# lhaippp/DMHomo

Hardware: AMD Instinct MI355X
Metric: sampled images/sec (128x128, s_step=32) (higher is better)
Workload: dtype f32; 1 GPU; DGM CFG-Unet dim=64 128x128 bs=25/GPU s_step=32 cond_scale=3 (BASELINE configs[1]); global_batch=25, cfg_mode=streams, hip_graph=True, weights=seeded random init

## Files before the change

### dmhomo_amd/_lib.py

```python
import contextlib
import ctypes as C
import gc
import os

import torch

_HERE = os.path.dirname(os.path.abspath(__file__))
LIB_PATH = os.environ.get('DMH_LIB_PATH') or os.path.join(_HERE, 'libdmhomo_hip.so')

c_f32p = C.c_void_p
c_i64 = C.c_int64
c_int = C.c_int
c_float = C.c_float


ABI_VERSION = 500


class DmhConv(C.Structure):
    _fields_ = [('struct_size', C.c_uint64)] + \
               [(n, C.c_void_p) for n in ('src0', 'src1', 'wpack', 'bias', 'in_coef', 'res', 'res_coef', 'out',
                                          'stats')] + \
               [(n, C.c_int32) for n in ('B', 'Hin', 'Win', 'C0', 'C1', 'Cout', 'KH', 'KW', 'stride', 'upsample2')] + \
               [('in_bound', C.c_void_p), ('in_bound_n', C.c_int32), ('fin_n', C.c_int32), ('fin_w', C.c_void_p),
                ('fin_b', C.c_void_p), ('fin_out', C.c_void_p), ('pix_stats', C.c_void_p), ('pix_eps', C.c_float),
                ('rows', C.c_void_p)]


class DmhPackJob(C.Structure):
    _fields_ = [('src', C.c_void_p), ('ws', C.c_void_p), ('wpack', C.c_void_p), ('Cout', C.c_int32), ('C0', C.c_int32),
                ('C1', C.c_int32), ('KH', C.c_int32), ('transposed', C.c_int32)]


class DmhStep(C.Structure):
    _fields_ = [('objective', C.c_int32), ('clip', C.c_int32), ('mode', C.c_int32), ('cond_scale', C.c_float),
                ('sqrt_recip_ac', C.c_float), ('sqrt_recipm1_ac', C.c_float), ('sqrt_ac', C.c_float),
                ('sqrt_1m_ac', C.c_float), ('c0', C.c_float), ('c1', C.c_float), ('c2', C.c_float)]


SIGNATURES = {
    'dmh_last_error': (C.c_char_p, []),
    'dmh_version': (c_int, []),
    'dmh_ws_standardize': (c_int, [c_f32p, c_f32p, c_int, c_int, c_float, C.c_void_p]),
    'dmh_conv_pack_floats': (c_i64, [c_int, c_int, c_int, c_int, c_int]),
    'dmh_pack_conv_weight': (c_int, [c_f32p, c_f32p, c_int, c_int, c_int, c_int, c_int, C.c_void_p]),
    'dmh_pack_conv_weights_multi': (c_int, [C.c_void_p, c_int, c_float, C.c_void_p]),
# ... 158 lines not shown
    'dmh_preview_sheet': (c_int, [c_f32p, c_f32p, c_f32p, C.c_void_p, C.c_void_p, c_int, c_int, c_int, c_int, c_int, c_int,
                                  C.c_void_p]),
    'dmh_homography_warp': (c_int, [c_f32p, C.c_void_p, c_f32p, c_int, c_int, c_int, c_int, c_int, C.c_void_p]),
    'dmh_hem_batch': (c_int, [C.c_void_p, C.c_void_p, C.c_void_p, C.c_void_p, C.c_void_p, C.c_void_p, c_int, c_int, c_int, c_int,
                              c_int, c_int, c_int, c_f32p, c_f32p, c_f32p, c_f32p, c_f32p, C.c_void_p]),
    'dmh_hem_flow': (c_int, [C.c_void_p, c_int, c_int, c_int, c_f32p, C.c_void_p]),
}

EXTENSIONS = {
    'dmh_known_blend': (c_int, [c_f32p, c_f32p, C.c_void_p, c_float, c_f32p, C.c_void_p, c_f32p, c_int, c_i64, C.c_void_p]),
    'dmh_known_error_splits': (c_int, [c_int, c_i64]),
    'dmh_known_error': (c_int, [c_f32p, c_f32p, C.c_void_p, c_float, c_f32p, C.c_void_p, C.c_void_p, C.c_void_p, c_int, c_i64,
                                C.c_void_p]),
}

DLT_BLOCKS = 64

_lib = None


class DmhError(RuntimeError):
    pass


def lib():
    global _lib
    if _lib is None:
        if not os.path.exists(LIB_PATH):
            raise DmhError(f'{LIB_PATH} not found: build it with `python -c "import __graft_entry__ as g; g.build()"` '
                           f'or `make -C dmhomo_amd/csrc` — dmhomo_amd has no CPU / eager fallback')
        h = C.CDLL(LIB_PATH)
        for name, (res, args) in list(SIGNATURES.items()) + list(EXTENSIONS.items()):
            fn = getattr(h, name)
            fn.restype = res
            fn.argtypes = args
        got = int(h.dmh_version())
        if got != ABI_VERSION:
            raise DmhError(f'{LIB_PATH} reports ABI version {got}, this binding was written against {ABI_VERSION} '
                           f'(include/dmhomo_hip.h): rebuild the library with `make -C dmhomo_amd/csrc`')
        _lib = h
    return _lib


def stream():
    return C.c_void_p(torch.cuda.current_stream().cuda_stream)


# ... 31 lines not shown
```

### dmhomo_amd/cfg.py

```python
import torch
from torch import nn

from . import _params as P
from . import ops
from .engine import UnetEngine
from .sampling import DeviceRng, ModelPrediction, ScheduleHost, default, exists, extract
from .schedule import make_buffers, ddim_pairs, linear_beta_schedule, cosine_beta_schedule


class Unet(nn.Module):

    def __init__(self, dim, num_classes, cond_drop_prob=0.5, init_dim=None, out_dim=None, dim_mults=(1, 2, 4, 8),
                 channels=3, resnet_block_groups=8, learned_variance=False, learned_sinusoidal_cond=False,
                 random_fourier_features=False, learned_sinusoidal_dim=16):
        super().__init__()
        self.cond_drop_prob = cond_drop_prob
        self.channels = channels
        input_channels = channels + 3
        init_dim = default(init_dim, dim)
        self.init_conv = nn.Conv2d(input_channels, init_dim, 7, padding=3)
        time_dim = dim * 4
        self.random_or_learned_sinusoidal_cond = learned_sinusoidal_cond or random_fourier_features
        pos_emb, fourier_dim = P.time_embedding(dim, learned_sinusoidal_cond, random_fourier_features, learned_sinusoidal_dim)
        self.time_mlp = nn.Sequential(pos_emb, nn.Linear(fourier_dim, time_dim), nn.GELU(), nn.Linear(time_dim, time_dim))
# ... 25 lines not shown
        z = cache.get(key)
        if z is None:
            z = cache[key] = torch.zeros((batch,), device=device, dtype=torch.uint8)
        return z

    def _stem(self, x, rgb_flow, mask):
        if not x.is_cuda:
            raise RuntimeError('dmhomo_amd.Unet runs on the GPU only (HIP kernels); move the inputs with .cuda()')
        eng = self._engine
        eng.ensure_prepared()
        xin = ops.assemble_input(x.to(torch.float32).contiguous(), rgb_flow.to(torch.float32).contiguous(),
                                 mask.to(torch.float32).contiguous(), reps=1, cpad=eng.cin_pad)
        return eng.stem(xin)

    def _run(self, x, time, classes, rgb_flow, mask, keeps, taps=None, x0=None, first=None, out=None, rows=None,
             x0_per_pass=False, pert_lo=None):
        eng = self._engine
        if x0 is None:
            x0 = self._stem(x, rgb_flow, mask)
        if len(keeps) > 1 and not x0_per_pass:
            x0 = x0.repeat(len(keeps), 1, 1, 1)
        time = time.to(torch.int64).contiguous()
        classes = classes.to(torch.int64).contiguous()
        tab = self.__dict__.get('_ss_tab')
        if tab is not None:
            T, Ct, cursor = tab
            B = classes.shape[0]
            ss_all = torch.empty((len(keeps) * B, T.shape[1]), device=T.device, dtype=torch.float32)
            for r, k in enumerate(keeps):
                ops.ss_gather(T, Ct, eng.mlp_b, cursor, classes, k, out=ss_all[r * B:(r + 1) * B])
            return eng.trunk(x0, None, taps, first=first, out=out, ss_all=ss_all, rows=rows, pert_lo=pert_lo)
        cond = eng.embed(time, [(classes, k) for k in keeps], len(keeps))
        return eng.trunk(x0, cond, taps, first=first, out=out, rows=rows, pert_lo=pert_lo)

    def forward(self, x, time, classes, rgb_flow, mask, cond_drop_prob=None):
        cond_drop_prob = default(cond_drop_prob, self.cond_drop_prob)
        keep = self._keep_mask(x.shape[0], cond_drop_prob, x.device)
        return self._run(x, time, classes, rgb_flow, mask, [keep])

    cfg_mode = 'batched'
    stream_splits = 1

    def _cond_null(self, x, time, classes, rgb_flow, mask, gate=None):
        B = x.shape[0]
        keep = self._keep_mask(B, self.cond_drop_prob, x.device)
        null = self._null_mask(B, x.device)
        dedup = bool(self.dedup_dropped_rows) and keep is not None
        if self.cfg_mode == 'streams':
            nsub = max(1, min(int(self.stream_splits), B))
            nstreams = 2 * nsub
            if len(getattr(self, '_side', ())) != nstreams:
                self._side = tuple(torch.cuda.Stream(device=x.device) for _ in range(nstreams))
            cur = torch.cuda.current_stream()
            x0 = self._stem(x, rgb_flow, mask)
            first = self._engine.first_conv(x0)
            cond_out = torch.empty((B, self.out_dim) + tuple(x.shape[2:]), device=x.device, dtype=torch.float32)
            null_out = torch.empty_like(cond_out)
            bounds = [(i * B) // nsub for i in range(nsub + 1)]
            si = 0
            for k, dst, sub, null_side in ((keep, cond_out, dedup, False), (null, null_out, False, True)):
                for lo, hi in zip(bounds[:-1], bounds[1:]):
                    st = self._side[si]
                    si += 1
                    st.wait_stream(cur)
                    with torch.cuda.stream(st):
                        kk = None if k is None else k[lo:hi].contiguous()
                        fs = None if first is None else (first[0][lo:hi], first[1][lo:hi])
                        if gate is not None:
                            rows = ops.rows_gated(kk if sub else None, hi - lo, 0, *gate, null_side=null_side)
                        else:
                            rows = ops.rows_from_keep(kk) if sub else None
                        self._run(None, time[lo:hi], classes[lo:hi], None, None, [kk], x0=x0[lo:hi], first=fs, out=dst[lo:hi],
                                  rows=rows)
            for st in self._side:
                cur.wait_stream(st)
            return cond_out, null_out, (keep if dedup else None)
        if gate is not None:
            rows = ops.rows_gated(keep if dedup else None, B, B, *gate)
        else:
            rows = ops.rows_from_keep(keep, extra=B) if dedup else None
        both = self._run(x, time, classes, rgb_flow, mask, [keep, null], rows=rows)
        return both[:B], both[B:], (keep if dedup else None)

    def _cond_null_noflow(self, x, time, classes, rgb_flow, mask, cond_scale):
        if self.cfg_mode == 'streams':
            raise ValueError("flow_guidance with cfg_mode = 'streams': the third pass is defined for cfg_mode = 'batched' only")
        B, eng = x.shape[0], self._engine
        keep = self._keep_mask(B, self.cond_drop_prob, x.device)
# ... 635 lines not shown
```

### dmhomo_amd/csrc/common.h

```cpp
#pragma once
#include <initializer_list>
#include <hip/hip_runtime.h>
#include <stdint.h>
#include <stdio.h>

#include "../../include/dmhomo_hip.h"

void dmh_set_error(const char* fmt, ...);

#define DMH_REQUIRE(cond, ...)   \
  do {                           \
    if (!(cond)) {               \
      dmh_set_error(__VA_ARGS__); \
      return DMH_EINVAL;         \
    }                            \
  } while (0)

#define DMH_CHECK_LAUNCH(name)                                        \
  do {                                                                \
    hipError_t e_ = hipGetLastError();                                \
    if (e_ != hipSuccess) {                                           \
      dmh_set_error("%s: launch failed: %s", name, hipGetErrorString(e_)); \
      return DMH_ELAUNCH;                                             \
    }                                                                 \
// ... 125 lines not shown
```

### dmhomo_amd/csrc/conv.hip

```cpp
#include <stdlib.h>

#include "common.h"

#include "conv_args.h"
#include "weight_image.h"

template <int KH, int KW, int S, int UPS, int KC, int TH, int TW>
struct ConvCfg {
  static constexpr int BM = TH * TW;
  static constexpr int MB = BM / 128;
  static constexpr int IN_H = (TH - 1) * S + KH;
  static constexpr int IN_W = (TW - 1) * S + KW;
  static constexpr int IN_PIX = IN_H * IN_W;
  static constexpr int KCP = KC + 4;
  static constexpr int C4 = KC / 4;
  static constexpr int NLOAD = (IN_PIX * C4 + 255) / 256;
  static constexpr int WL = 64 * C4 / 256;
  static constexpr int PAD = (S == 1) ? (KH / 2) : (KH == 4 ? 1 : 0);
  static constexpr int IN_FLOATS = IN_PIX * KCP;
  static constexpr int W_FLOATS = 64 * KCP;
  static constexpr int EPI_BYTES = 4 * 32 * 68 * 4;
  static constexpr int MAIN_BYTES = (IN_FLOATS + 2 * W_FLOATS) * 4;
  static constexpr int LDS_BYTES = MAIN_BYTES > EPI_BYTES ? MAIN_BYTES : EPI_BYTES;
};
// ... 296 lines not shown
  DMH_REQUIRE(w && wpack && dmh_conv_up2_pack_floats(Cout, C0) > 0, "dmh_pack_conv_weight_up2: bad arguments");
  return dmh_f16x3_up2_pack(w, wpack, Cout, C0, (hipStream_t)stream);
}

extern "C" int dmh_pack_conv_weights_multi(const DmhPackJob* jobs, int njobs, float ws_eps, void* stream) {
  DMH_REQUIRE(jobs && njobs > 0, "dmh_pack_conv_weights_multi: bad arguments");
  DMH_REQUIRE(conv3_variant() == 9, "dmh_pack_conv_weights_multi: only the fp16-piece images (DMH_CONV3_VARIANT=9)");
  for (int i = 0; i < njobs; ++i) {
    const DmhPackJob& j = jobs[i];
    DMH_REQUIRE(j.src && j.wpack && j.Cout > 0 && j.C0 > 0 && j.C1 >= 0 && (j.KH == 1 || j.KH == 3) &&
                    (j.transposed == 0 || (j.transposed == 1 && j.C1 == 0)),
                "dmh_pack_conv_weights_multi: job %d: stride-1 1x1 / 3x3 weights only (Cout %d, C0 %d, C1 %d, KH %d, transposed %d)",
                i, j.Cout, j.C0, j.C1, j.KH, j.transposed);
  }
  return dmh_f16x3_pack_multi(jobs, njobs, ws_eps, (hipStream_t)stream);
}

extern "C" int dmh_ws_standardize(const float* w, float* w_out, int Cout, int K, float eps, void* stream) {
  DMH_REQUIRE(w && w_out && Cout > 0 && K > 0, "dmh_ws_standardize: bad arguments");
  hipLaunchKernelGGL(ws_standardize_kernel, dim3(Cout), dim3(256), 0, (hipStream_t)stream, w, w_out, K, eps);
  DMH_CHECK_LAUNCH("dmh_ws_standardize");
  return DMH_OK;
}

extern "C" int dmh_conv2d(const DmhConv* d, void* stream) {
  DMH_REQUIRE(d && d->struct_size == sizeof(DmhConv),
              "dmh_conv2d: DmhConv.struct_size is %llu, this library's DmhConv has %llu bytes (header / library mismatch)",
              d ? (unsigned long long)d->struct_size : 0ull, (unsigned long long)sizeof(DmhConv));
  DMH_REQUIRE(d->src0 && d->wpack, "dmh_conv2d: null pointer");
  DMH_REQUIRE(d->B > 0 && d->Hin > 0 && d->Win > 0 && d->C0 > 0 && d->Cout > 0, "dmh_conv2d: bad shape");
// ... 62 lines not shown
```

### dmhomo_amd/csrc/conv_args.h

```cpp
#pragma once
#include "common.h"

typedef float floatx16 __attribute__((ext_vector_type(16)));

struct ConvArgs {
  const float* src0;
  const float* src1;
  const float* wpack;
  const float* bias;
  const float* in_coef;
  const float* res;
  const float* res_coef;
  float* out;
  float* stats;
  const float* oscale;
  const float* in_bound;
  int in_bound_n;
  int fin_n;
  const float* fin_w;
  const float* fin_b;
  float* fin_out;
  float* pix_stats;
  float pix_eps;
  int B, Hin, Win, C0, C1, Cout, Hout, Wout;
  int nch0, nch1, tilesX, tilesY;
  int ablate;
  int xcd;
  const int32_t* rows;
};


static inline ConvArgs fill_conv_args(const DmhConv* d, int Hout, int Wout, int KC, int TH, int TW) {
  ConvArgs a;
  a.src0 = d->src0;
  a.src1 = d->src1;
  a.wpack = d->wpack;
  a.bias = d->bias;
  a.in_coef = d->in_coef;
  a.res = d->res;
  a.res_coef = d->res_coef;
  a.out = d->out;
  a.stats = d->stats;
  a.oscale = nullptr;
// ... 8 lines not shown
  a.B = d->B;
  a.Hin = d->Hin;
  a.Win = d->Win;
  a.C0 = d->C0;
  a.C1 = d->src1 ? d->C1 : 0;
  a.Cout = d->Cout;
  a.Hout = Hout;
  a.Wout = Wout;
  a.nch0 = cdiv(a.C0, KC);
  a.nch1 = cdiv(a.C1, KC);
  a.tilesX = cdiv(Wout, TW);
  a.tilesY = cdiv(Hout, TH);
  a.ablate = 0;
  a.xcd = 1;
  a.rows = d->rows;
  return a;
}


int64_t dmh_wino_pack_floats(int Cout, int C0, int C1);
int dmh_wino_pack(const float* w, float* wpack, int Cout, int C0, int C1, hipStream_t st);
int dmh_wino_launch(const DmhConv* d, int Hout, int Wout, hipStream_t st);


int64_t dmh_f16x3_pack_floats(int Cout, int C0, int C1, int KH, int KW);
int dmh_f16x3_pack(const float* w, float* wpack, int Cout, int C0, int C1, int KH, int KW, hipStream_t st);
int dmh_f16x3_launch(const DmhConv* d, int Hout, int Wout, hipStream_t st);
int dmh_f16x3_pack_multi(const DmhPackJob* jobs, int njobs, float eps, hipStream_t st);
int64_t dmh_f16x3_up2_pack_floats(int Cout, int C0);
int dmh_f16x3_up2_pack(const float* w, float* wpack, int Cout, int C0, hipStream_t st);
int dmh_f16x3_launch_up2(const DmhConv* d, int Hout, int Wout, hipStream_t st);


struct EpilogueRows {
  static constexpr int EP = 68;
  int b, n0, chn, c4, rsub;
  bool cok;
  float4 bias, ra, rb, s1, s2, osc;

  __device__ __forceinline__ EpilogueRows(const ConvArgs& p, int b_, int n0_) : b(b_), n0(n0_) {
    const int lane = threadIdx.x & 63;
    c4 = lane & 15;
    rsub = lane >> 4;
// ... 218 lines not shown
```

### dmhomo_amd/csrc/conv_f16x3.hip

```cpp
#include <stdlib.h>

#include "common.h"

#include "conv_args.h"
#include "weight_image.h"

typedef _Float16 half8 __attribute__((ext_vector_type(8)));
typedef _Float16 half4 __attribute__((ext_vector_type(4)));
typedef float float4v __attribute__((ext_vector_type(4)));

namespace {

constexpr int KC = 32;
constexpr int PITCH = 160;
constexpr int STEP_U4 = 4 * 64;

template <int KH, int KW, int S, int UPS, int TH, int TW, int WM, int WN>
struct F16Cfg {
  static_assert(WM * WN == 4, "four waves per workgroup");
  static constexpr bool SUB = UPS == 3;
  static_assert(SUB || TH * TW == WM * 64, "64 pixels per wave");
  static_assert(!SUB || (KH == 2 && KW == 2 && S == 1 && TH == 4 && TW == 16 && WM == 4 && WN == 1), "sub-pixel geometry");
  static constexpr int IN_H = SUB ? TH + 2 : (TH - 1) * S + KH;
  static constexpr int IN_W = SUB ? TW + 2 : (TW - 1) * S + KW;
// ... 4 lines not shown
  static constexpr int ROWP = IN_W * PITCH;
  static constexpr int IN_BYTES = IN_H * ROWP;
  static constexpr int EPI_BYTES = 4 * 32 * EpilogueRows::EP * 4;
  static constexpr int TILE_BYTES = IN_BYTES > EPI_BYTES ? IN_BYTES : EPI_BYTES;
  static constexpr int LDS_BYTES = TILE_BYTES + 16;
};

__device__ __forceinline__ unsigned absbits(float x) { return __float_as_uint(x) & 0x7fffffffu; }

__device__ __forceinline__ int64_t f16x3_frag_floats_dev(int Cout, int C0, int C1, int T) {
  return (int64_t)((Cout + 63) / 64) * ((C0 + KC - 1) / KC + (C1 + KC - 1) / KC) * T * 2 * STEP_U4 * 4;
}

}

template <int KH, int KW, int S, int UPS, int TH, int TW, int WM, int WN>
__global__ __launch_bounds__(256, 2) void conv_f16x3_kernel(ConvArgs p) {
  using Cfg = F16Cfg<KH, KW, S, UPS, TH, TW, WM, WN>;
  constexpr bool PK = UPS == 4;
  constexpr int IN_W = Cfg::IN_W, IN_PIX = Cfg::IN_PIX, NLOAD = Cfg::NLOAD, NTAPS = PK ? (KH * KW + 1) / 2 : KH * KW,
                ROWP = Cfg::ROWP;

  extern __shared__ __attribute__((aligned(16))) float lds[];
  unsigned char* in_tile = reinterpret_cast<unsigned char*>(lds);
  unsigned* mxslot = reinterpret_cast<unsigned*>(in_tile + Cfg::TILE_BYTES);

  const int tid = threadIdx.x;
  const int lane = tid & 63;
  const int wave = tid >> 6;
  const int wave_u = __builtin_amdgcn_readfirstlane(wave);
  const int kg = lane >> 4;
  const int l15 = lane & 15;
  const int wm = wave / WN, wn = wave % WN;
// ... 346 lines not shown
#pragma unroll
    for (int mb = 0; mb < 4; mb += 2)
      asm volatile("s_nop 15" : "+v"(acc[mb][0]), "+v"(acc[mb][1]), "+v"(acc[mb][2]), "+v"(acc[mb][3]), "+v"(acc[mb + 1][0]),
                   "+v"(acc[mb + 1][1]), "+v"(acc[mb + 1][2]), "+v"(acc[mb + 1][3]));
    __builtin_amdgcn_sched_barrier(0);
    STAMP(4)
  }

#ifdef DMH_STAMPS
  if (!(p.ablate & 4))
#endif
  {
    constexpr int EP = EpilogueRows::EP;
    const float inv_s = __uint_as_float((unsigned)(e_run - 14) << 23);
    float* wl = lds + wave * (32 * EP);
    EpilogueRows er(p, b, n0);
    if (UPS == 3 && p.oscale) er.osc = ld4(p.oscale + nt * 64 + er.c4 * 4);
    er.osc.x *= inv_s;
    er.osc.y *= inv_s;
    er.osc.z *= inv_s;
    er.osc.w *= inv_s;
    __syncthreads();
#pragma unroll
    for (int hb = 0; hb < 2; ++hb) {
#pragma unroll
      for (int m2 = 0; m2 < 2; ++m2)
#pragma unroll
        for (int nb = 0; nb < 4; ++nb)
          *reinterpret_cast<float4v*>(wl + (m2 * 16 + l15) * EP + nb * 16 + kg * 4) = acc[hb * 2 + m2][nb];
      __builtin_amdgcn_fence(__ATOMIC_RELEASE, "wavefront");
      __builtin_amdgcn_wave_barrier();
      __builtin_amdgcn_fence(__ATOMIC_ACQUIRE, "wavefront");
      if (UPS == 3) er.template store_rows<TW>(p, wl, hb * 32, oy0, ox0, 2, wm >> 1, wm & 1);
      else er.template store_rows<TW, (KH == 1 && KW == 1 && WN == 1 && UPS == 0)>(p, wl, wm * 64 + hb * 32, oy0, ox0);
    }
#ifdef DMH_STAMPS
    STAMP(5)
    if (p.stats && lane == 0 && by == 0) {
      const int stiles = ((p.Hout + 7) / 8) * p.tilesX;
      unsigned long long* d = reinterpret_cast<unsigned long long*>(
                                  p.stats + ((size_t)(b * stiles + (ty * (TH / 8)) * p.tilesX + tx) * p.Cout) * 2) + wave * 8;
      for (int i = 0; i < 6; ++i) d[i] = tk[i];
      d[6] = t_now - t_begin;
      d[7] = __builtin_amdgcn_s_memrealtime() - rt_begin;
    }
#else
    er.template write_stats_grid<WM, WN, TH>(p, lds, ty, tx, by);
#endif
  }
}
#undef STAMP

__global__ __launch_bounds__(64) void f16x3_wscale_kernel(const float* __restrict__ w, float* __restrict__ oscale,
                                                           int Cout, int K) {
  const int o = blockIdx.x;
  float m = 0.f;
  if (o < Cout)
    for (int i = threadIdx.x; i < K; i += 64) m = fmaxf(m, fabsf(w[(size_t)o * K + i]));
  const float s = f16x3_row_scale(m);
  if (threadIdx.x == 0) oscale[o] = s;
}

// ... 11 lines not shown
    if (s.o < Cout) ws = w[((size_t)s.o * C0 + cr) * 16 + ky * 4 + kx] / oscale[s.o];
  } else {
    const int tt = 2 * s.tap + (s.k >> 4), cc = s.k & 15;
    if (s.o < Cout && cc < C0 && tt < 49) ws = w[((size_t)s.o * C0 + cc) * 49 + tt] / oscale[s.o];
  }
  wp[idx] = f16x3_piece(ws, s.plane);
}

static int64_t f16x3_frag_floats(int Cout, int C0, int C1, int KH, int KW);
#define PM_MAX 32
struct PmTable {
  const float* src[PM_MAX];
  float* ws[PM_MAX];
  float* wpack[PM_MAX];
  int Cout[PM_MAX], C0[PM_MAX], C1[PM_MAX], T[PM_MAX], tr[PM_MAX];
  int blk0[PM_MAX + 1];
  int count;
};
__device__ __forceinline__ int pm_find(const PmTable& t, int blk) {
  int lo = 0, hi = t.count;
  while (hi - lo > 1) {
    const int mid = (lo + hi) >> 1;
    if (t.blk0[mid] <= blk) lo = mid; else hi = mid;
  }
  return lo;
}
__device__ __forceinline__ float pm_elem(const float* w, int o, int c, int tap, int Cout, int Cin, int T, int tr) {
  return tr ? w[((size_t)c * Cout + o) * T + (T - 1 - tap)] : w[((size_t)o * Cin + c) * T + tap];
}
__global__ __launch_bounds__(256) void pm_ws_kernel(PmTable t, float eps) {
  const int ti = pm_find(t, blockIdx.x), o = blockIdx.x - t.blk0[ti];
  const int K = (t.tr[ti] ? t.Cout[ti] : t.C0[ti] + t.C1[ti]) * t.T[ti];
  ws_standardize_row(t.src[ti] + (size_t)o * K, t.ws[ti] + (size_t)o * K, K, eps);
}
__global__ __launch_bounds__(64) void pm_wscale_kernel(PmTable t) {
  const int ti = pm_find(t, blockIdx.x), o = blockIdx.x - t.blk0[ti];
  const int Cout = t.Cout[ti], Cin = t.C0[ti] + t.C1[ti], T = t.T[ti], tr = t.tr[ti], K = Cin * T;
  const float* w = t.ws[ti] ? t.ws[ti] : t.src[ti];
  float m = 0.f;
  if (o < Cout)
    for (int i = threadIdx.x; i < K; i += 64) m = fmaxf(m, fabsf(pm_elem(w, o, i / T, i % T, Cout, Cin, T, tr)));
  const float sc = f16x3_row_scale(m);
  if (threadIdx.x == 0) t.wpack[ti][f16x3_frag_floats_dev(Cout, t.C0[ti], t.C1[ti], T) + o] = sc;
}
__global__ __launch_bounds__(256) void pm_pack_kernel(PmTable t) {
  const int ti = pm_find(t, blockIdx.x);
  const int Cout = t.Cout[ti], C0 = t.C0[ti], C1 = t.C1[ti], T = t.T[ti], tr = t.tr[ti];
  const int nch0 = (C0 + KC - 1) / KC, nch1 = (C1 + KC - 1) / KC;
  const int64_t frag = f16x3_frag_floats_dev(Cout, C0, C1, T);
  const int64_t total = frag * 2;
  const float* w = t.ws[ti] ? t.ws[ti] : t.src[ti];
  const float* oscale = t.wpack[ti] + frag;
  _Float16* wp = reinterpret_cast<_Float16*>(t.wpack[ti]);
  const int64_t base = (int64_t)(blockIdx.x - t.blk0[ti]) * 2048;
  for (int64_t idx = base + threadIdx.x; idx < min(base + 2048, total); idx += 256) {
    const F16x3Slot s = f16x3_slot(idx, T, nch0 + nch1);
    const bool src1 = s.ch >= nch0;
    const int c = (s.ch - (src1 ? nch0 : 0)) * KC + s.k;
    float ws = 0.f;
    if (c < (src1 ? C1 : C0) && s.o < Cout)
      ws = pm_elem(w, s.o, c + (src1 ? C0 : 0), s.tap, Cout, C0 + C1, T, tr) / oscale[s.o];
    wp[idx] = f16x3_piece(ws, s.plane);
  }
}

int dmh_f16x3_pack_multi(const DmhPackJob* jobs, int njobs, float eps, hipStream_t st) {
  for (int phase = 0; phase < 3; ++phase) {
    for (int i0 = 0; i0 < njobs;) {
      PmTable t;
      int k = 0, blocks = 0;
      for (; k < PM_MAX && i0 < njobs; ++i0) {
        const DmhPackJob& j = jobs[i0];
        if (phase == 0 && !j.ws) continue;
        const int T = j.KH * j.KH;
        t.src[k] = j.src;
        t.ws[k] = j.ws;
        t.wpack[k] = j.wpack;
        t.Cout[k] = j.Cout;
        t.C0[k] = j.C0;
        t.C1[k] = j.C1;
        t.T[k] = T;
        t.tr[k] = j.transposed;
        t.blk0[k] = blocks;
        if (phase == 0) blocks += j.transposed ? j.C0 + j.C1 : j.Cout;
        else if (phase == 1) blocks += cdiv(j.Cout, 64) * 64;
        else blocks += (int)cdiv64(f16x3_frag_floats(j.Cout, j.C0, j.C1, j.KH, j.KH) * 2, 2048);
        ++k;
      }
      if (k == 0) continue;
      t.blk0[k] = blocks;
      t.count = k;
      if (phase == 0) hipLaunchKernelGGL(pm_ws_kernel, dim3(blocks), dim3(256), 0, st, t, eps);
      else if (phase == 1) hipLaunchKernelGGL(pm_wscale_kernel, dim3(blocks), dim3(64), 0, st, t);
      else hipLaunchKernelGGL(pm_pack_kernel, dim3(blocks), dim3(256), 0, st, t);
      DMH_CHECK_LAUNCH("dmh_pack_conv_weights_multi");
    }
  }
  return DMH_OK;
}

static bool f16x3_pk(int C0, int C1, int KH) { return KH == 7 && C1 == 0 && C0 <= 16; }

static int64_t f16x3_frag_floats(int Cout, int C0, int C1, int KH, int KW) {
  if (KH == 4) return (int64_t)cdiv(Cout, 64) * (4 * C0 / KC) * 4 * 2 * STEP_U4 * 4;
  if (f16x3_pk(C0, C1, KH)) return (int64_t)cdiv(Cout, 64) * 25 * 2 * STEP_U4 * 4;
  return (int64_t)cdiv(Cout, 64) * (cdiv(C0, KC) + cdiv(C1, KC)) * KH * KW * 2 * STEP_U4 * 4;
}

int64_t dmh_f16x3_pack_floats(int Cout, int C0, int C1, int KH, int KW) {
  return f16x3_frag_floats(Cout, C0, C1, KH, KW) + (int64_t)cdiv(Cout, 64) * 64;
}

int dmh_f16x3_pack(const float* w, float* wpack, int Cout, int C0, int C1, int KH, int KW, hipStream_t st) {
  const bool s2d = KH == 4;
  if (!s2d && !f16x3_pk(C0, C1, KH)) {
// ... 64 lines not shown

int dmh_f16x3_launch_up2(const DmhConv* d, int Hout, int Wout, hipStream_t st) {
  using Cfg = F16Cfg<2, 2, 1, 3, 4, 16, 4, 1>;
  ConvArgs a = fill_conv_args(d, Hout, Wout, KC, 4, 16);
  a.tilesX = cdiv(d->Win, 16);
  a.tilesY = cdiv(d->Hin, 4);
  a.oscale = d->wpack + f16x3_frag_floats(4 * d->Cout, a.C0, 0, 2, 2);
  auto kern = conv_f16x3_kernel<2, 2, 1, 3, 4, 16, 4, 1>;
  DMH_RAISE_LDS_ONCE(kern, Cfg::LDS_BYTES, "dmh_conv2d(f16x3 sub-pixel)");
  dim3 grid(a.tilesX * a.tilesY * a.B, cdiv(a.Cout, 64));
  hipLaunchKernelGGL(kern, grid, dim3(256), Cfg::LDS_BYTES, st, a);
  DMH_CHECK_LAUNCH("dmh_conv2d(f16x3 sub-pixel)");
  return DMH_OK;
}

int dmh_f16x3_launch(const DmhConv* d, int Hout, int Wout, hipStream_t st) {
  const bool wide = d->Cout % 128 == 0;
  if (d->KH == 4) {
    return wide ? launch_f16x3<2, 2, 1, 2, 8, 16, 2, 2>(d, Hout, Wout, st)
                : launch_f16x3<2, 2, 1, 2, 16, 16, 4, 1>(d, Hout, Wout, st);
  }
  if (d->KH == 7) {
    if (f16x3_pk(d->C0, d->src1 ? d->C1 : 0, 7)) return launch_f16x3<7, 7, 1, 4, 16, 16, 4, 1>(d, Hout, Wout, st);
    return launch_f16x3<7, 7, 1, 0, 16, 16, 4, 1>(d, Hout, Wout, st);
  }
  if (d->KH == 1) {
    return wide ? launch_f16x3<1, 1, 1, 0, 8, 16, 2, 2>(d, Hout, Wout, st)
                : launch_f16x3<1, 1, 1, 0, 16, 16, 4, 1>(d, Hout, Wout, st);
  }
  if (d->upsample2) {
// ... 8 lines not shown
```

### dmhomo_amd/engine.py

```python
import torch

from . import ops
from .layout import ATTN_SCALE, HIDDEN, sinusoidal_freq, unet_layout

FUSED_FINAL = True


class _Res:
    __slots__ = ('conv1', 'g1', 'b1', 'conv2', 'g2', 'b2', 'res', 'ss_off', 'cout')


class _Attn:
    __slots__ = ('linear', 'ln_g', 'qkv', 'pla', 'plo', 'out', 'out_g')


class UnetEngine:
    def __init__(self, module, groups=8):
        self.module = module
        self.groups = groups
        self._sig = None
        self._rows = None
        self._pert_lo = None

    def _signature(self):
# ... 68 lines not shown
            return a

        self.blocks = []
        for n in L.nodes:
            k = n.keys
            if n.kind == 'res':
                b = res(n)
            elif n.kind in ('linattn', 'attn'):
                b = attn(n)
            elif n.kind == 'unshuffle':
                w22 = f32(k['w']).reshape(n.cout, n.c0, 2, 2).contiguous()
                b = ops.PackedConv(w22, f32(k['b']), n.c0, 0, stride=2, batch=pb)
            else:
                b = conv(k['w'], k['b'], n.c0, stride=2 if n.kind == 'down4' else 1, ups=1 if n.kind == 'up3' else 0)
            self.blocks.append((n, b))
        pb.run()
        nxt = [b for _, b in self.blocks[1:]] + [None]
        self._pixel_stats = [isinstance(a, _Attn) and a.pla is not None for a in nxt]
        self.final_w = f32('final_conv.weight').reshape(L.out_dim, -1).contiguous()
        self.final_b = f32('final_conv.bias')
        res_nodes = [n for n in L.nodes if n.kind == 'res']
        self.mlp_wt = torch.cat([f32(n.keys['mlp_w']).t() for n in res_nodes], dim=1).contiguous()
        self.mlp_b = torch.cat([f32(n.keys['mlp_b']) for n in res_nodes]).contiguous()

    def _res(self, r, x0, x1, ss_all, pixel_stats=False, pre=None, final=None, keep_out=True, fin_out=None):
        B, H, W, _ = x0.shape
        hw = H * W
        rows = self._rows
        y1, st1 = pre if pre is not None else ops.conv2d(r.conv1, x0, x1, want_stats=True, rows=rows)
        ss = ss_all[:, r.ss_off:r.ss_off + 2 * r.cout]
        coef1, bound1 = ops.gn_finalize(st1, r.g1, r.b1, hw, self.groups, ss, want_bound=True, rows=rows)
        y2, st2 = ops.conv2d(r.conv2, y1, in_coef=coef1, want_stats=True, in_bound=bound1, rows=rows)
        coef2 = ops.gn_finalize(st2, r.g2, r.b2, hw, self.groups, rows=rows)
        if final is not None:
            return ops.conv2d(r.res, x0, x1, res=y2, res_coef=coef2, final=final, keep_out=keep_out, fin_out=fin_out, rows=rows)
        if r.res is not None:
            if pixel_stats and r.cout == 64 and r.res.k == 1 and ops.f16x3_default():
                return ops.conv2d(r.res, x0, x1, res=y2, res_coef=coef2, pixel_stats=True, rows=rows)
            x = ops.conv2d(r.res, x0, x1, res=y2, res_coef=coef2, rows=rows)
            return (x, None) if pixel_stats else x
        assert x1 is None
        if pixel_stats:
            if r.cout in ops.PIXEL_STATS_FUSABLE:
                return ops.gn_silu_residual(y2, coef2, x0, pixel_stats=True, rows=rows)
# ... 45 lines not shown
        cond_t[:, td:].zero_()
        cond_c = self.embed(torch.zeros((ncls + 1,), dtype=torch.int64, device=dev), [(cls, keep)], 1)
        cond_c[:, :td].zero_()
        T = ops.linear(cond_t, self.mlp_wt, None, act_in='silu')
        Ct = ops.linear(cond_c, self.mlp_wt, None, act_in='silu')
        return T, Ct

    def stem(self, xin):
        self.ensure_prepared()
        return ops.conv2d(self.init_conv, xin)

    def first_conv(self, x0):
        self.ensure_prepared()
        return ops.conv2d(self.blocks[0][1].conv1, x0, None, want_stats=True)

    def trunk(self, x0, cond, taps=None, first=None, out=None, ss_all=None, rows=None, pert_lo=None):
        self.ensure_prepared()
        self._rows, self._pert_lo = rows, pert_lo
        try:
            return self._trunk(x0, cond, taps, first, out, ss_all)
        finally:
            self._rows = self._pert_lo = None

    def _trunk(self, x0, cond, taps, first, out, ss_all):
        rows = self._rows

        def tap(name, v):
            if taps is not None:
                taps[name] = v
            return v
        if ss_all is None:
            ss_all = ops.linear(cond, self.mlp_wt, self.mlp_b, act_in='silu')
        x = tap('init_conv', x0)
        hs, pst, last = [x], None, len(self.blocks) - 1
        for i, (n, b) in enumerate(self.blocks):
            x1 = hs.pop() if n.c1 else None
            if n.kind == 'res':
                if i == last and FUSED_FINAL and b.res is not None and b.res.k == 1 and b.cout <= 64 \
                        and self.final_w.shape[0] <= 8 and ops.f16x3_default():
                    x, y = self._res(b, x, x1, ss_all, final=(self.final_w, self.final_b), keep_out=taps is not None,
                                     fin_out=out)
                    tap(n.name, x)
                    return y
                if self._pixel_stats[i]:
                    x, pst = self._res(b, x, x1, ss_all, pixel_stats=True)
                else:
                    x = self._res(b, x, x1, ss_all, pre=first if i == 0 else None)
            elif n.kind in ('linattn', 'attn'):
                x, pst = self._attn(b, x, pst), None
            else:
                x = ops.conv2d(b, x, rows=rows)
            tap(n.name, x)
            if n.push:
                hs.append(x)
        y = ops.final_conv_nchw(x, self.final_w, self.final_b)
        if out is not None:
            out.copy_(y)
            return out
        return y
```

### dmhomo_amd/ops.py

```python
import ctypes as C
import math

import os

import torch

from . import _lib
from ._lib import call, ptr, lib

F32 = torch.float32


def _empty(shape, like, dtype=F32):
    return torch.empty(shape, device=like.device, dtype=dtype)


def ws_standardize(w, eps=1e-5, out=None):
    w = w.detach().contiguous()
    out = torch.empty_like(w) if out is None else out
    cout = w.shape[0]
    call('dmh_ws_standardize', ptr(w), ptr(out), cout, w.numel() // cout, float(eps))
    return out


class PackBatch:

    def __init__(self):
        self.jobs, self.pre, self.specials, self._keep, self._arr = [], [], [], [], None

    def add(self, src, ws, wpack, cout, c0, c1, kh, transposed):
        self.jobs.append(_lib.DmhPackJob(ptr(src), ptr(ws), ptr(wpack), cout, c0, c1, kh, int(transposed)))
        self._keep.append((src, ws, wpack))
        self._arr = None

    def run(self, eps=1e-5):
        for f in self.pre:
            f()
        if self.jobs:
            if self._arr is None:
                self._arr = (_lib.DmhPackJob * len(self.jobs))(*self.jobs)
            call('dmh_pack_conv_weights_multi', C.cast(self._arr, C.c_void_p), len(self.jobs), float(eps))
        for f in self.specials:
            f()


def f16x3_default():
    return os.environ.get('DMH_CONV3_VARIANT', '9') == '9'


class PackedConv:
    __slots__ = ('wpack', 'bias', 'cout', 'c0', 'c1', 'k', 'stride', 'upsample2', '_w', '_up2')

    def __init__(self, w_oihw, bias, c0, c1=0, stride=1, upsample2=0, subpixel=True, batch=None, ws_from=None,
                 transposed=False):
        w = w_oihw.detach()
        assert w.is_contiguous()
# ... 21 lines not shown
        else:
            if src is not None:
                batch.pre.append(lambda: ws_standardize(src, out=w))
            if transposed:
                self._w = wt = _empty((cout, cin, kh, kw), w)
                batch.pre.append(lambda: wt.copy_(w.flip(2, 3).transpose(0, 1)))
            batch.specials.append(self.repack)
        if own:
            batch.run()

    def repack(self):
        if self._up2:
            call('dmh_pack_conv_weight_up2', ptr(self._w), ptr(self.wpack), self.cout, self.c0)
        else:
            call('dmh_pack_conv_weight', ptr(self._w), ptr(self.wpack), self.cout, self.c0, self.c1, self.k, self.k)


def conv_out_hw(pc, h, w):
    if pc.upsample2:
        return h * 2, w * 2
    if pc.stride == 2:
        return h // 2, w // 2
    return h, w


CONV_LOG = None


def rows_from_keep(keep, extra=0):
    B = keep.shape[0]
# ... 1276 lines not shown
```

Measured before the change: 89.57 images/s.

## Stack first and last res-block 3x3 convs over shared stem input

The last up-block res conv1 concatenates its skip with the stem output x0. Its x0 part is now computed once per step together with the first block's conv1 in a stacked 128-channel conv kernel. The tail conv then only covers the remaining channels and adds the precomputed partial as a residual. This removes redundant work on x0 and one full 3x3 pass over those channels. In exchange it adds a new packing path, a templated epilogue branch and repeats for CFG passes.

Result: no change. 89.96 images/s, median of 6 (+0.4%).

```diff
diff --git a/dmhomo_amd/_lib.py b/dmhomo_amd/_lib.py
--- a/dmhomo_amd/_lib.py
+++ b/dmhomo_amd/_lib.py
@@ -30,6 +30,11 @@
 class DmhPackJob(C.Structure):
     _fields_ = [('src', C.c_void_p), ('ws', C.c_void_p), ('wpack', C.c_void_p), ('Cout', C.c_int32), ('C0', C.c_int32),
                 ('C1', C.c_int32), ('KH', C.c_int32), ('transposed', C.c_int32)]
+
+
+class DmhPackPart(C.Structure):
+    _fields_ = [('src', C.c_void_p), ('wpack', C.c_void_p)] + \
+               [(n, C.c_int32) for n in ('Cout', 'C0', 'KH', 'src_cin', 'src_c0', 'img_cout', 'img_o0')]
 
 
 class DmhStep(C.Structure):
@@ -218,6 +223,11 @@
                                 C.c_void_p]),
 }
 
+HEAD_ENTRIES = {
+    'dmh_pack_conv_weight_parts': (c_int, [C.c_void_p, c_int, C.c_void_p]),
+    'dmh_conv2d_stacked': (c_int, [C.POINTER(DmhConv), c_f32p, c_int, C.c_void_p]),
+}
+
 DLT_BLOCKS = 64
 
 _lib = None
@@ -234,7 +244,7 @@
             raise DmhError(f'{LIB_PATH} not found: build it with `python -c "import __graft_entry__ as g; g.build()"` '
                            f'or `make -C dmhomo_amd/csrc` — dmhomo_amd has no CPU / eager fallback')
         h = C.CDLL(LIB_PATH)
-        for name, (res, args) in list(SIGNATURES.items()) + list(EXTENSIONS.items()):
+        for name, (res, args) in list(SIGNATURES.items()) + list(EXTENSIONS.items()) + list(HEAD_ENTRIES.items()):
             fn = getattr(h, name)
             fn.restype = res
             fn.argtypes = args
diff --git a/dmhomo_amd/cfg.py b/dmhomo_amd/cfg.py
--- a/dmhomo_amd/cfg.py
+++ b/dmhomo_amd/cfg.py
@@ -63,10 +63,17 @@
         return eng.stem(xin)
 
     def _run(self, x, time, classes, rgb_flow, mask, keeps, taps=None, x0=None, first=None, out=None, rows=None,
-             x0_per_pass=False, pert_lo=None):
+             x0_per_pass=False, pert_lo=None, partial=None):
         eng = self._engine
         if x0 is None:
             x0 = self._stem(x, rgb_flow, mask)
+        if first is None and partial is None:
+            head = eng.shared_head(x0)
+            if head is not None:
+                first, partial = head[:2], head[2]
+                if len(keeps) > 1 and not x0_per_pass:
+                    first = tuple(v.repeat(len(keeps), 1, 1, 1) for v in first)
+                    partial = partial.repeat(len(keeps), 1, 1, 1)
         if len(keeps) > 1 and not x0_per_pass:
             x0 = x0.repeat(len(keeps), 1, 1, 1)
         time = time.to(torch.int64).contiguous()
@@ -78,9 +85,10 @@
             ss_all = torch.empty((len(keeps) * B, T.shape[1]), device=T.device, dtype=torch.float32)
             for r, k in enumerate(keeps):
                 ops.ss_gather(T, Ct, eng.mlp_b, cursor, classes, k, out=ss_all[r * B:(r + 1) * B])
-            return eng.trunk(x0, None, taps, first=first, out=out, ss_all=ss_all, rows=rows, pert_lo=pert_lo)
+            return eng.trunk(x0, None, taps, first=first, out=out, ss_all=ss_all, rows=rows, pert_lo=pert_lo,
+                             skip_partial=partial)
         cond = eng.embed(time, [(classes, k) for k in keeps], len(keeps))
-        return eng.trunk(x0, cond, taps, first=first, out=out, rows=rows, pert_lo=pert_lo)
+        return eng.trunk(x0, cond, taps, first=first, out=out, rows=rows, pert_lo=pert_lo, skip_partial=partial)
 
     def forward(self, x, time, classes, rgb_flow, mask, cond_drop_prob=None):
         cond_drop_prob = default(cond_drop_prob, self.cond_drop_prob)
@@ -102,7 +110,8 @@
                 self._side = tuple(torch.cuda.Stream(device=x.device) for _ in range(nstreams))
             cur = torch.cuda.current_stream()
             x0 = self._stem(x, rgb_flow, mask)
-            first = self._engine.first_conv(x0)
+            head = self._engine.shared_head(x0)
+            first, part = (head[:2], head[2]) if head is not None else (self._engine.first_conv(x0), None)
             cond_out = torch.empty((B, self.out_dim) + tuple(x.shape[2:]), device=x.device, dtype=torch.float32)
             null_out = torch.empty_like(cond_out)
             bounds = [(i * B) // nsub for i in range(nsub + 1)]
@@ -120,7 +129,7 @@
                         else:
                             rows = ops.rows_from_keep(kk) if sub else None
                         self._run(None, time[lo:hi], classes[lo:hi], None, None, [kk], x0=x0[lo:hi], first=fs, out=dst[lo:hi],
-                                  rows=rows)
+                                  rows=rows, partial=None if part is None else part[lo:hi])
             for st in self._side:
                 cur.wait_stream(st)
             return cond_out, null_out, (keep if dedup else None)
diff --git a/dmhomo_amd/csrc/common.h b/dmhomo_amd/csrc/common.h
--- a/dmhomo_amd/csrc/common.h
+++ b/dmhomo_amd/csrc/common.h
@@ -5,6 +5,7 @@
 #include <stdio.h>
 
 #include "../../include/dmhomo_hip.h"
+#include "../../include/dmhomo_hip_head.h"
 
 void dmh_set_error(const char* fmt, ...);
 
diff --git a/dmhomo_amd/csrc/conv.hip b/dmhomo_amd/csrc/conv.hip
--- a/dmhomo_amd/csrc/conv.hip
+++ b/dmhomo_amd/csrc/conv.hip
@@ -334,6 +334,38 @@
                 i, j.Cout, j.C0, j.C1, j.KH, j.transposed);
   }
   return dmh_f16x3_pack_multi(jobs, njobs, ws_eps, (hipStream_t)stream);
+}
+
+extern "C" int dmh_pack_conv_weight_parts(const DmhPackPart* parts, int nparts, void* stream) {
+  DMH_REQUIRE(parts && nparts > 0, "dmh_pack_conv_weight_parts: bad arguments");
+  DMH_REQUIRE(conv3_variant() == 9, "dmh_pack_conv_weight_parts: only the fp16-piece images (DMH_CONV3_VARIANT=9)");
+  for (int i = 0; i < nparts; ++i) {
+    const DmhPackPart& q = parts[i];
+    DMH_REQUIRE(q.src && q.wpack && dmh_dims_ok({q.Cout, q.C0, q.src_cin, q.img_cout}) && (q.KH == 1 || q.KH == 3) &&
+                    q.src_c0 >= 0 && q.src_c0 <= q.src_cin - q.C0 && q.img_o0 >= 0 && q.img_o0 % 64 == 0 &&
+                    q.img_o0 <= q.img_cout - q.Cout,
+                "dmh_pack_conv_weight_parts: part %d: stride-1 1x1 / 3x3 weights, input channels inside the source, output "
+                "channels from a multiple of 64 inside the image (Cout %d, C0 %d, KH %d, source %d + %d, image %d + %d)",
+                i, q.Cout, q.C0, q.KH, q.src_cin, q.src_c0, q.img_cout, q.img_o0);
+  }
+  return dmh_f16x3_pack_parts(parts, nparts, (hipStream_t)stream);
+}
+
+extern "C" int dmh_conv2d_stacked(const DmhConv* d, float* out2, int Cout2, void* stream) {
+  DMH_REQUIRE(d && d->struct_size == sizeof(DmhConv),
+              "dmh_conv2d_stacked: DmhConv.struct_size is %llu, this library's DmhConv has %llu bytes (header / library mismatch)",
+              d ? (unsigned long long)d->struct_size : 0ull, (unsigned long long)sizeof(DmhConv));
+  DMH_REQUIRE(d->src0 && d->wpack && d->out && out2, "dmh_conv2d_stacked: null pointer");
+  DMH_REQUIRE(conv3_variant() == 9, "dmh_conv2d_stacked: only the fp16-piece kernels (DMH_CONV3_VARIANT=9)");
+  DMH_REQUIRE(dmh_dims_ok({d->B, d->Hin, d->Win, d->C0, d->Cout, Cout2}) && (int64_t)d->B * d->Hin * d->Win < ((int64_t)1 << 31),
+              "dmh_conv2d_stacked: bad shape");
+  DMH_REQUIRE(d->C0 % 4 == 0 && d->Cout % 4 == 0 && Cout2 % 4 == 0 && d->Cout <= 64 && Cout2 <= 64,
+              "dmh_conv2d_stacked: channels must be multiples of 4, at most 64 per output (got %d -> %d, %d)", d->C0, d->Cout,
+              Cout2);
+  DMH_REQUIRE(d->KH == 3 && d->KW == 3 && d->stride == 1 && d->upsample2 == 0 && !d->src1 && !d->in_coef && !d->in_bound &&
+                  !d->res && !d->res_coef && !d->fin_w && !d->pix_stats,
+              "dmh_conv2d_stacked: a plain stride-1 3x3 over one source (no prologue, residual, projection or pixel statistics)");
+  return dmh_f16x3_launch_stacked(d, out2, Cout2, d->Hin, d->Win, (hipStream_t)stream);
 }
 
 extern "C" int dmh_ws_standardize(const float* w, float* w_out, int Cout, int K, float eps, void* stream) {
diff --git a/dmhomo_amd/csrc/conv_args.h b/dmhomo_amd/csrc/conv_args.h
--- a/dmhomo_amd/csrc/conv_args.h
+++ b/dmhomo_amd/csrc/conv_args.h
@@ -27,6 +27,8 @@
   int ablate;
   int xcd;
   const int32_t* rows;
+  float* out2;
+  int Cout2;
 };
 
 
@@ -65,6 +67,8 @@
   a.ablate = 0;
   a.xcd = 1;
   a.rows = d->rows;
+  a.out2 = nullptr;
+  a.Cout2 = 0;
   return a;
 }
 
@@ -78,6 +82,8 @@
 int dmh_f16x3_pack(const float* w, float* wpack, int Cout, int C0, int C1, int KH, int KW, hipStream_t st);
 int dmh_f16x3_launch(const DmhConv* d, int Hout, int Wout, hipStream_t st);
 int dmh_f16x3_pack_multi(const DmhPackJob* jobs, int njobs, float eps, hipStream_t st);
+int dmh_f16x3_pack_parts(const DmhPackPart* parts, int nparts, hipStream_t st);
+int dmh_f16x3_launch_stacked(const DmhConv* d, float* out2, int Cout2, int Hout, int Wout, hipStream_t st);
 int64_t dmh_f16x3_up2_pack_floats(int Cout, int C0);
 int dmh_f16x3_up2_pack(const float* w, float* wpack, int Cout, int C0, hipStream_t st);
 int dmh_f16x3_launch_up2(const DmhConv* d, int Hout, int Wout, hipStream_t st);
diff --git a/dmhomo_amd/csrc/conv_f16x3.hip b/dmhomo_amd/csrc/conv_f16x3.hip
--- a/dmhomo_amd/csrc/conv_f16x3.hip
+++ b/dmhomo_amd/csrc/conv_f16x3.hip
@@ -42,9 +42,10 @@
 
 }
 
-template <int KH, int KW, int S, int UPS, int TH, int TW, int WM, int WN>
+template <int KH, int KW, int S, int UPS, int TH, int TW, int WM, int WN, bool STK = false>
 __global__ __launch_bounds__(256, 2) void conv_f16x3_kernel(ConvArgs p) {
   using Cfg = F16Cfg<KH, KW, S, UPS, TH, TW, WM, WN>;
+  static_assert(!STK || (WN == 2 && UPS == 0), "the stacked launch is two 64-channel wave columns");
   constexpr bool PK = UPS == 4;
   constexpr int IN_W = Cfg::IN_W, IN_PIX = Cfg::IN_PIX, NLOAD = Cfg::NLOAD, NTAPS = PK ? (KH * KW + 1) / 2 : KH * KW,
                 ROWP = Cfg::ROWP;
@@ -421,7 +422,19 @@
     constexpr int EP = EpilogueRows::EP;
     const float inv_s = __uint_as_float((unsigned)(e_run - 14) << 23);
     float* wl = lds + wave * (32 * EP);
-    EpilogueRows er(p, b, n0);
+    ConvArgs ps;
+    if constexpr (STK) {
+      ps = p;
+      ps.Cout = wn ? p.Cout2 : p.Cout;
+      ps.out = wn ? p.out2 : p.out;
+      ps.bias = wn ? nullptr : p.bias;
+      ps.oscale = p.oscale + n0;
+    }
+    const ConvArgs& q = [&]() -> const ConvArgs& {
+      if constexpr (STK) return ps;
+      else return p;
+    }();
+    EpilogueRows er(q, b, STK ? 0 : n0);
     if (UPS == 3 && p.oscale) er.osc = ld4(p.oscale + nt * 64 + er.c4 * 4);
     er.osc.x *= inv_s;
     er.osc.y *= inv_s;
@@ -438,8 +451,8 @@
       __builtin_amdgcn_fence(__ATOMIC_RELEASE, "wavefront");
       __builtin_amdgcn_wave_barrier();
       __builtin_amdgcn_fence(__ATOMIC_ACQUIRE, "wavefront");
-      if (UPS == 3) er.template store_rows<TW>(p, wl, hb * 32, oy0, ox0, 2, wm >> 1, wm & 1);
-      else er.template store_rows<TW, (KH == 1 && KW == 1 && WN == 1 && UPS == 0)>(p, wl, wm * 64 + hb * 32, oy0, ox0);
+      if (UPS == 3) er.template store_rows<TW>(q, wl, hb * 32, oy0, ox0, 2, wm >> 1, wm & 1);
+      else er.template store_rows<TW, (KH == 1 && KW == 1 && WN == 1 && UPS == 0)>(q, wl, wm * 64 + hb * 32, oy0, ox0);
     }
 #ifdef DMH_STAMPS
     STAMP(5)
@@ -452,7 +465,7 @@
       d[7] = __builtin_amdgcn_s_memrealtime() - rt_begin;
     }
 #else
-    er.template write_stats_grid<WM, WN, TH>(p, lds, ty, tx, by);
+    er.template write_stats_grid<WM, WN, TH>(q, lds, ty, tx, by);
 #endif
   }
 }
@@ -494,6 +507,7 @@
   float* ws[PM_MAX];
   float* wpack[PM_MAX];
   int Cout[PM_MAX], C0[PM_MAX], C1[PM_MAX], T[PM_MAX], tr[PM_MAX];
+  int sCin[PM_MAX], sc0[PM_MAX], icout[PM_MAX], o0[PM_MAX];
   int blk0[PM_MAX + 1];
   int count;
 };
@@ -519,19 +533,19 @@
   const float* w = t.ws[ti] ? t.ws[ti] : t.src[ti];
   float m = 0.f;
   if (o < Cout)
-    for (int i = threadIdx.x; i < K; i += 64) m = fmaxf(m, fabsf(pm_elem(w, o, i / T, i % T, Cout, Cin, T, tr)));
+    for (int i = threadIdx.x; i < K; i += 64)
+      m = fmaxf(m, fabsf(pm_elem(w, o, t.sc0[ti] + i / T, i % T, Cout, t.sCin[ti], T, tr)));
   const float sc = f16x3_row_scale(m);
-  if (threadIdx.x == 0) t.wpack[ti][f16x3_frag_floats_dev(Cout, t.C0[ti], t.C1[ti], T) + o] = sc;
+  if (threadIdx.x == 0) t.wpack[ti][f16x3_frag_floats_dev(t.icout[ti], t.C0[ti], t.C1[ti], T) + t.o0[ti] + o] = sc;
 }
 __global__ __launch_bounds__(256) void pm_pack_kernel(PmTable t) {
   const int ti = pm_find(t, blockIdx.x);
   const int Cout = t.Cout[ti], C0 = t.C0[ti], C1 = t.C1[ti], T = t.T[ti], tr = t.tr[ti];
   const int nch0 = (C0 + KC - 1) / KC, nch1 = (C1 + KC - 1) / KC;
-  const int64_t frag = f16x3_frag_floats_dev(Cout, C0, C1, T);
-  const int64_t total = frag * 2;
+  const int64_t total = f16x3_frag_floats_dev(Cout, C0, C1, T) * 2;
   const float* w = t.ws[ti] ? t.ws[ti] : t.src[ti];
-  const float* oscale = t.wpack[ti] + frag;
-  _Float16* wp = reinterpret_cast<_Float16*>(t.wpack[ti]);
+  const float* oscale = t.wpack[ti] + f16x3_frag_floats_dev(t.icout[ti], C0, C1, T) + t.o0[ti];
+  _Float16* wp = reinterpret_cast<_Float16*>(t.wpack[ti] + f16x3_frag_floats_dev(t.o0[ti], C0, C1, T));
   const int64_t base = (int64_t)(blockIdx.x - t.blk0[ti]) * 2048;
   for (int64_t idx = base + threadIdx.x; idx < min(base + 2048, total); idx += 256) {
     const F16x3Slot s = f16x3_slot(idx, T, nch0 + nch1);
@@ -539,12 +553,12 @@
     const int c = (s.ch - (src1 ? nch0 : 0)) * KC + s.k;
     float ws = 0.f;
     if (c < (src1 ? C1 : C0) && s.o < Cout)
-      ws = pm_elem(w, s.o, c + (src1 ? C0 : 0), s.tap, Cout, C0 + C1, T, tr) / oscale[s.o];
+      ws = pm_elem(w, s.o, t.sc0[ti] + c + (src1 ? C0 : 0), s.tap, Cout, t.sCin[ti], T, tr) / oscale[s.o];
     wp[idx] = f16x3_piece(ws, s.plane);
   }
 }
 
-int dmh_f16x3_pack_multi(const DmhPackJob* jobs, int njobs, float eps, hipStream_t st) {
+static int f16x3_pack_table(const DmhPackJob* jobs, const DmhPackPart* parts, int njobs, float eps, hipStream_t st) {
   for (int phase = 0; phase < 3; ++phase) {
     for (int i0 = 0; i0 < njobs;) {
       PmTable t;
@@ -552,6 +566,10 @@
       for (; k < PM_MAX && i0 < njobs; ++i0) {
         const DmhPackJob& j = jobs[i0];
         if (phase == 0 && !j.ws) continue;
+        t.sCin[k] = parts ? parts[i0].src_cin : j.C0 + j.C1;
+        t.sc0[k] = parts ? parts[i0].src_c0 : 0;
+        t.icout[k] = parts ? parts[i0].img_cout : j.Cout;
+        t.o0[k] = parts ? parts[i0].img_o0 : 0;
         const int T = j.KH * j.KH;
         t.src[k] = j.src;
         t.ws[k] = j.ws;
@@ -579,6 +597,24 @@
   return DMH_OK;
 }
 
+int dmh_f16x3_pack_multi(const DmhPackJob* jobs, int njobs, float eps, hipStream_t st) {
+  return f16x3_pack_table(jobs, nullptr, njobs, eps, st);
+}
+
+int dmh_f16x3_pack_parts(const DmhPackPart* parts, int nparts, hipStream_t st) {
+  for (int i0 = 0; i0 < nparts; i0 += PM_MAX) {
+    DmhPackJob jobs[PM_MAX];
+    const int n = nparts - i0 < PM_MAX ? nparts - i0 : PM_MAX;
+    for (int i = 0; i < n; ++i) {
+      const DmhPackPart& q = parts[i0 + i];
+      jobs[i] = DmhPackJob{q.src, nullptr, q.wpack, q.Cout, q.C0, 0, q.KH, 0};
+    }
+    const int rc = f16x3_pack_table(jobs, parts + i0, n, 0.f, st);
+    if (rc != DMH_OK) return rc;
+  }
+  return DMH_OK;
+}
+
 static bool f16x3_pk(int C0, int C1, int KH) { return KH == 7 && C1 == 0 && C0 <= 16; }
 
 static int64_t f16x3_frag_floats(int Cout, int C0, int C1, int KH, int KW) {
@@ -673,6 +709,20 @@
   return DMH_OK;
 }
 
+int dmh_f16x3_launch_stacked(const DmhConv* d, float* out2, int Cout2, int Hout, int Wout, hipStream_t st) {
+  using Cfg = F16Cfg<3, 3, 1, 0, 8, 16, 2, 2>;
+  ConvArgs a = fill_conv_args(d, Hout, Wout, KC, 8, 16);
+  a.oscale = d->wpack + f16x3_frag_floats(128, a.C0, 0, 3, 3);
+  a.out2 = out2;
+  a.Cout2 = Cout2;
+  auto kern = conv_f16x3_kernel<3, 3, 1, 0, 8, 16, 2, 2, true>;
+  DMH_RAISE_LDS_ONCE(kern, Cfg::LDS_BYTES, "dmh_conv2d_stacked");
+  dim3 grid(a.tilesX * a.tilesY * a.B, 1);
+  hipLaunchKernelGGL(kern, grid, dim3(256), Cfg::LDS_BYTES, st, a);
+  DMH_CHECK_LAUNCH("dmh_conv2d_stacked");
+  return DMH_OK;
+}
+
 int dmh_f16x3_launch(const DmhConv* d, int Hout, int Wout, hipStream_t st) {
   const bool wide = d->Cout % 128 == 0;
   if (d->KH == 4) {
diff --git a/dmhomo_amd/engine.py b/dmhomo_amd/engine.py
--- a/dmhomo_amd/engine.py
+++ b/dmhomo_amd/engine.py
@@ -106,6 +106,7 @@
             else:
                 b = conv(k['w'], k['b'], n.c0, stride=2 if n.kind == 'down4' else 1, ups=1 if n.kind == 'up3' else 0)
             self.blocks.append((n, b))
+        self._shared_head(pb)
         pb.run()
         nxt = [b for _, b in self.blocks[1:]] + [None]
         self._pixel_stats = [isinstance(a, _Attn) and a.pla is not None for a in nxt]
@@ -115,11 +116,26 @@
         self.mlp_wt = torch.cat([f32(n.keys['mlp_w']).t() for n in res_nodes], dim=1).contiguous()
         self.mlp_b = torch.cat([f32(n.keys['mlp_b']) for n in res_nodes]).contiguous()
 
-    def _res(self, r, x0, x1, ss_all, pixel_stats=False, pre=None, final=None, keep_out=True, fin_out=None):
+    def _shared_head(self, pb):
+        self.head = self.head_x = None
+        (n0, first), (nl, last) = self.blocks[0], self.blocks[-1]
+        if not (ops.f16x3_default() and len(self.blocks) > 1 and n0.kind == 'res' and nl.kind == 'res' and not n0.c1):
+            return
+        c = n0.c0
+        if not (nl.c1 == c and first.conv1.k == 3 and last.conv1.k == 3 and first.cout <= 64 and last.cout <= 64):
+            return
+        self.head = ops.PackedStacked((first.conv1._w, 0), (last.conv1._w, nl.c0), c, first.conv1.bias, pb)
+        self.head_x = ops.packed_conv_part(last.conv1._w, 0, nl.c0, last.conv1.bias, pb)
+
+    def _res(self, r, x0, x1, ss_all, pixel_stats=False, pre=None, final=None, keep_out=True, fin_out=None, partial=None):
         B, H, W, _ = x0.shape
         hw = H * W
         rows = self._rows
-        y1, st1 = pre if pre is not None else ops.conv2d(r.conv1, x0, x1, want_stats=True, rows=rows)
+        if partial is not None:
+            assert pre is None and x1 is not None and partial.shape == (B, H, W, r.cout), (partial.shape, x0.shape)
+            y1, st1 = ops.conv2d(self.head_x, x0, res=partial, want_stats=True, rows=rows)
+        else:
+            y1, st1 = pre if pre is not None else ops.conv2d(r.conv1, x0, x1, want_stats=True, rows=rows)
         ss = ss_all[:, r.ss_off:r.ss_off + 2 * r.cout]
         coef1, bound1 = ops.gn_finalize(st1, r.g1, r.b1, hw, self.groups, ss, want_bound=True, rows=rows)
         y2, st2 = ops.conv2d(r.conv2, y1, in_coef=coef1, want_stats=True, in_bound=bound1, rows=rows)
@@ -195,15 +211,21 @@
         self.ensure_prepared()
         return ops.conv2d(self.blocks[0][1].conv1, x0, None, want_stats=True)
 
-    def trunk(self, x0, cond, taps=None, first=None, out=None, ss_all=None, rows=None, pert_lo=None):
+    def shared_head(self, x0):
+        self.ensure_prepared()
+        if self.head is None:
+            return None
+        return ops.conv2d_stacked(self.head, x0)
+
+    def trunk(self, x0, cond, taps=None, first=None, out=None, ss_all=None, rows=None, pert_lo=None, skip_partial=None):
         self.ensure_prepared()
         self._rows, self._pert_lo = rows, pert_lo
         try:
-            return self._trunk(x0, cond, taps, first, out, ss_all)
+            return self._trunk(x0, cond, taps, first, out, ss_all, skip_partial)
         finally:
             self._rows = self._pert_lo = None
 
-    def _trunk(self, x0, cond, taps, first, out, ss_all):
+    def _trunk(self, x0, cond, taps, first, out, ss_all, skip_partial=None):
         rows = self._rows
 
         def tap(name, v):
@@ -216,17 +238,21 @@
         hs, pst, last = [x], None, len(self.blocks) - 1
         for i, (n, b) in enumerate(self.blocks):
             x1 = hs.pop() if n.c1 else None
+            part = None
+            if i == last and skip_partial is not None:
+                assert self.head_x is not None and n.kind == 'res' and x1 is x0
+                part = skip_partial
             if n.kind == 'res':
                 if i == last and FUSED_FINAL and b.res is not None and b.res.k == 1 and b.cout <= 64 \
                         and self.final_w.shape[0] <= 8 and ops.f16x3_default():
                     x, y = self._res(b, x, x1, ss_all, final=(self.final_w, self.final_b), keep_out=taps is not None,
-                                     fin_out=out)
+                                     fin_out=out, partial=part)
                     tap(n.name, x)
                     return y
                 if self._pixel_stats[i]:
                     x, pst = self._res(b, x, x1, ss_all, pixel_stats=True)
                 else:
-                    x = self._res(b, x, x1, ss_all, pre=first if i == 0 else None)
+                    x = self._res(b, x, x1, ss_all, pre=first if i == 0 else None, partial=part)
             elif n.kind in ('linattn', 'attn'):
                 x, pst = self._attn(b, x, pst), None
             else:
diff --git a/dmhomo_amd/ops.py b/dmhomo_amd/ops.py
--- a/dmhomo_amd/ops.py
+++ b/dmhomo_amd/ops.py
@@ -27,11 +27,18 @@
 
     def __init__(self):
         self.jobs, self.pre, self.specials, self._keep, self._arr = [], [], [], [], None
+        self.parts, self._parr = [], None
 
     def add(self, src, ws, wpack, cout, c0, c1, kh, transposed):
         self.jobs.append(_lib.DmhPackJob(ptr(src), ptr(ws), ptr(wpack), cout, c0, c1, kh, int(transposed)))
         self._keep.append((src, ws, wpack))
         self._arr = None
+
+    def add_part(self, src, src_c0, c0, wpack, img_cout, img_o0):
+        cout, cin, kh, _ = src.shape
+        self.parts.append(_lib.DmhPackPart(ptr(src), ptr(wpack), cout, c0, kh, cin, src_c0, img_cout, img_o0))
+        self._keep.append((src, wpack))
+        self._parr = None
 
     def run(self, eps=1e-5):
         for f in self.pre:
@@ -40,6 +47,10 @@
             if self._arr is None:
                 self._arr = (_lib.DmhPackJob * len(self.jobs))(*self.jobs)
             call('dmh_pack_conv_weights_multi', C.cast(self._arr, C.c_void_p), len(self.jobs), float(eps))
+        if self.parts:
+            if self._parr is None:
+                self._parr = (_lib.DmhPackPart * len(self.parts))(*self.parts)
+            call('dmh_pack_conv_weight_parts', C.cast(self._parr, C.c_void_p), len(self.parts))
         for f in self.specials:
             f()
 
@@ -91,6 +102,43 @@
             call('dmh_pack_conv_weight_up2', ptr(self._w), ptr(self.wpack), self.cout, self.c0)
         else:
             call('dmh_pack_conv_weight', ptr(self._w), ptr(self.wpack), self.cout, self.c0, self.c1, self.k, self.k)
+
+
+def packed_conv_part(src, src_c0, c0, bias, batch):
+    assert f16x3_default() and src.is_contiguous() and src.shape[2] == src.shape[3] and src.shape[2] in (1, 3), src.shape
+    assert 0 <= src_c0 and src_c0 + c0 <= src.shape[1], (src.shape, src_c0, c0)
+    pc = PackedConv.__new__(PackedConv)
+    pc._w, pc._up2 = src, False
+    pc.cout, pc.c0, pc.c1, pc.k, pc.stride, pc.upsample2 = src.shape[0], c0, 0, src.shape[2], 1, 0
+    pc.wpack = _empty((lib().dmh_conv_pack_floats(pc.cout, c0, 0, pc.k, pc.k),), src)
+    pc.bias = None if bias is None else bias.detach().contiguous()
+    batch.add_part(src, src_c0, c0, pc.wpack, pc.cout, 0)
+    return pc
+
+
+class PackedStacked:
+    __slots__ = ('wpack', 'bias', 'c0', 'cout', 'cout2')
+
+    def __init__(self, a, b, c0, bias, batch):
+        (wa, a0), (wb, b0) = a, b
+        assert f16x3_default() and wa.shape[2:] == (3, 3) and wb.shape[2:] == (3, 3), (wa.shape, wb.shape)
+        assert wa.shape[0] <= 64 and wb.shape[0] <= 64, (wa.shape, wb.shape)
+        self.c0, self.cout, self.cout2 = c0, wa.shape[0], wb.shape[0]
+        self.wpack = _empty((lib().dmh_conv_pack_floats(128, c0, 0, 3, 3),), wa)
+        self.bias = None if bias is None else bias.detach().contiguous()
+        batch.add_part(wa, a0, c0, self.wpack, 128, 0)
+        batch.add_part(wb, b0, c0, self.wpack, 128, 64)
+
+
+def conv2d_stacked(ps, src0, rows=None):
+    B, H, W, c0 = src0.shape
+    assert c0 == ps.c0, (src0.shape, ps.c0)
+    out, out2 = _empty((B, H, W, ps.cout), src0), _empty((B, H, W, ps.cout2), src0)
+    stats = _empty((B, lib().dmh_conv_tiles(H, W, 3, 1), ps.cout, 2), src0)
+    d = _lib.DmhConv(C.sizeof(_lib.DmhConv), ptr(src0), None, ptr(ps.wpack), ptr(ps.bias), None, None, None, ptr(out), ptr(stats),
+                     B, H, W, c0, 0, ps.cout, 3, 3, 1, 0, None, 0, 0, None, None, None, None, 0., _rows(rows))
+    call('dmh_conv2d_stacked', C.byref(d), ptr(out2), ps.cout2)
+    return out, stats, out2
 
 
 def conv_out_hw(pc, h, w):
diff --git a/include/dmhomo_hip_head.h b/include/dmhomo_hip_head.h
--- /dev/null
+++ b/include/dmhomo_hip_head.h
@@ -0,0 +1,26 @@
+#ifndef DMHOMO_HIP_HEAD_H
+#define DMHOMO_HIP_HEAD_H
+
+#include <stdint.h>
+
+#include "dmhomo_hip.h"
+
+#ifdef __cplusplus
+extern "C" {
+#endif
+
+typedef struct DmhPackPart {
+  const float* src;
+  float* wpack;
+  int32_t Cout, C0, KH;
+  int32_t src_cin, src_c0;
+  int32_t img_cout, img_o0;
+} DmhPackPart;
+int dmh_pack_conv_weight_parts(const DmhPackPart* parts, int nparts, void* stream);
+
+int dmh_conv2d_stacked(const DmhConv* d, float* out2, int Cout2, void* stream);
+
+#ifdef __cplusplus
+}
+#endif
+#endif
```
